# nk35jk/Chainer_Realtime_Multi-Person_Pose_Estimation

Measured on AMD Instinct MI355X. Metric: frames/sec end-to-end (CNN+PAF grouping) at 368×368, 1/2/4/8 MI355X, higher is better.
Workload: dtype bf16x3 (hi/lo split operands, f32 accumulate); 1 GPU; 368x368 frames, full PoseDetector.__call__ path (upload, resize+normalise, 92-conv CocoPoseNet in bf16x3: 3xBF16 split products, f32 accumulate, PAF post-process), batch of 232 frames per GPU per step; net_input=368x368, heatmap=320x320, maps=synthetic

## Files before the change

chainer_realtime_multi-person_pose_estimation_amd/_lib.py:

```python
import ctypes
import os

import numpy as np

_HERE = os.path.dirname(os.path.abspath(__file__))
LIB_PATH = os.path.join(_HERE, "libopenpose_hip%s.so" % (
    "." + os.environ["OP_LIB_VARIANT"] if os.environ.get("OP_LIB_VARIANT") else ""))

OP_OK, OP_ERR_INVALID, OP_ERR_HIP, OP_ERR_CAPACITY, OP_ERR_INDEX, OP_ERR_STATE, OP_ERR_TIMEOUT = range(7)
OP_COMM_ID_BYTES = 128
N_JOINTS, N_LIMBS, N_PAF, N_HEAT, N_LAYERS = 18, 19, 38, 19, 92

EXPORTED = (
    "op_last_error", "op_build_info", "op_default_params", "op_default_limits", "op_layer_info", "op_create", "op_destroy",
    "op_set_weights", "op_detect", "op_preprocess", "op_forward", "op_forward_stages", "op_forward_probe",
    "op_forward_probe_info", "op_resize_images", "op_compute_peaks",
    "op_compute_connections", "op_grouping", "op_postprocess", "op_stage_frames", "op_stage_maps",
    "op_use_staged_maps", "op_run_staged", "op_run_staged_graph", "op_graph_info", "op_synchronize", "op_fetch_result",
    "op_last_timing", "op_forward_flops", "op_profile_enable", "op_profile_read", "op_profile_reset",
    "op_set_precision", "op_get_precision", "op_fetch_results", "op_fetch_maps", "op_upload_frames", "op_upload_wait", "op_conv_census", "op_host_alloc", "op_host_free",
    "op_pack_results", "op_comm_unique_id", "op_comm_create", "op_comm_destroy", "op_comm_gather_results",
    "op_comm_wait", "op_comm_overflow", "op_comm_overflow_result", "op_detect_precise", "op_resize_cubic",
    "op_set_conv_algo", "op_set_stage_layout", "op_set_batch_invariant", "op_set_peak_mode", "op_profile_classes", "op_run_staged_precise",
    "op_cpm_layer_count", "op_cpm_layer_info", "op_cpm_create", "op_cpm_destroy", "op_cpm_set_weights",
# ... 309 lines not shown
        p.n_scales = len(sc)
        for i, v in enumerate(sc):
            p.inference_scales[i] = float(v)
    if "limbs_point" in d:
        for i, (a, b) in enumerate(d["limbs_point"]):
            p.limbs_point[i][0] = int(a)
            p.limbs_point[i][1] = int(b)
    return p


def layer_table():
    out = []
    name = ctypes.c_char_p()
    ci, co, k = ctypes.c_int32(), ctypes.c_int32(), ctypes.c_int32()
    for i in range(N_LAYERS):
        check(lib().op_layer_info(i, ctypes.byref(name), ctypes.byref(ci), ctypes.byref(co), ctypes.byref(k)))
        out.append((name.value.decode(), ci.value, co.value, k.value))
    return out


N_PROBE_POINTS = 46


def probe_table():
    out = []
    name = ctypes.c_char_p()
    ch, div = ctypes.c_int32(), ctypes.c_int32()
    for i in range(N_PROBE_POINTS):
        check(lib().op_forward_probe_info(i, ctypes.byref(name), ctypes.byref(ch), ctypes.byref(div)),
              "op_forward_probe_info")
        out.append((name.value.decode(), ch.value, div.value))
    return out


N_TRAIN_BUFFERS = 89


def train_buffer_table():
    out = []
    name = ctypes.c_char_p()
    ch, div = ctypes.c_int32(), ctypes.c_int32()
    for i in range(N_TRAIN_BUFFERS):
        check(lib().op_train_buffer_info(i, ctypes.byref(name), ctypes.byref(ch), ctypes.byref(div)),
              "op_train_buffer_info")
        out.append((name.value.decode(), ch.value, div.value))
    return out


CENSUS = {"7x7_splitk": 11, "7x7_other": 12, "3x3_w48": 13, "3x3_w32": 14, "3x3_pool": 15, "3x3_splitk": 16,
          "3x3_big": 17, "conv1_pair": 18, "3x3_r256": 19, "3x3_r128": 20, "3x3_r_pool": 21,
          "7x7_planar": 22, "7x7_frame_aligned": 23, "7x7_tight": 24,
          "cubic_fused": 25, "cubic_two_pass": 26,
          "cubic_rows": 28, "f32_lds": 29, "7x7_stag": 30, "7x7_plain_ring": 31,
          "7x7_q": 32, "7x7_circ": 33, "precise_side": 34, "7x7_q_iwg": 35, "7x7_lin": 36, "7x7_q_bpf": 37, "7x7_pers": 38}
CENSUS_SLOTS = 40


def conv_census(reset=False):
    a = (ctypes.c_int32 * CENSUS_SLOTS)()
    check(lib().op_conv_census(a, CENSUS_SLOTS, 1 if reset else 0), "op_conv_census")
    out = {"npx": {i: a[i] for i in range(1, 11) if a[i]}}
    out.update({k: a[v] for k, v in CENSUS.items()})
    return out


def forward_flops(h, w):
    return float(lib().op_forward_flops(int(h), int(w)))


class Context(object):

    def __init__(self, device=0, params=None, limits=None):
        L = lib()
        self._p = params if params is not None else default_params()
        self._l = limits if limits is not None else OpLimits()
        h = ctypes.c_void_p()
        check(L.op_create(ctypes.byref(self._p), ctypes.byref(self._l), int(device), ctypes.byref(h)), "op_create")
        self.h = h
        self.device = device

    def close(self):
        if getattr(self, "h", None) is not None and self.h.value:
            lib().op_destroy(self.h)
            self.h = None

    def __del__(self):
        try:
            self.close()
        except Exception:
            pass

    def set_precision(self, mode):
        check(lib().op_set_precision(self.h, PRECISION[mode]), "op_set_precision")

    def get_precision(self):
        m = ctypes.c_int32()
        check(lib().op_get_precision(self.h, ctypes.byref(m)), "op_get_precision")
        return {v: k for k, v in PRECISION.items()}[m.value]

    def set_weights(self, weights):
        table = layer_table()
        keep = []
        Wp = (ctypes.c_void_p * N_LAYERS)()
        bp = (ctypes.c_void_p * N_LAYERS)()
        for i, (name, ci, co, k) in enumerate(table):
            if name not in weights:
                raise KeyError("missing weights for layer %s" % name)
# ... 1077 lines not shown
```

chainer_realtime_multi-person_pose_estimation_amd/csrc/conv_big.hip:

```cpp
#include <atomic>
#include <array>
#include <map>
#include <mutex>
#include <tuple>
#include <cstdlib>
#include <vector>

#include "conv_big.hpp"
#include "conv_m16k.hpp"

namespace op {


template <int NPB, int KS, int PLANE_W>
__device__ __forceinline__ void big_taps(int nt, floatx16 (&acc)[2][NPB], const char* bp0, int hplane,
                                         const uint32_t (&qp)[(NPB + 1) / 2], const char* wb0, const char* wb1,
                                         int t, int pitch, int hi) {
  bf16x8g bh[2], bl[2], ah[2], al[2];
  auto q0 = [&](int pb) -> int { return (int)((qp[pb >> 1] >> (16 * (pb & 1))) & 0xffffu); };
  int toff = (t / KS) * pitch + (t - (t / KS) * KS);
  bh[0] = *(const bf16x8g*)(bp0 + (q0(0) + toff) * 16);
  bl[0] = *(const bf16x8g*)(bp0 + hplane + (q0(0) + toff) * 16);
#pragma unroll 1
  for (int u = 0; u < nt; ++u) {
// ... 889 lines not shown
      }
      if (plain_order) {
        tl.xpu = 0;
        tl.pair = 1;
      }
      tl.zeros = device_zeros();
      const char* trim_env = getenv("OP_M16_TRIM");
      tl.halo_trim = !(trim_env && atoi(trim_env) == 0);
      if (!tl.zeros) {
        set_error("conv_m16_bf16x3: conv_big_device_init was not called for this device");
        return OP_ERR_STATE;
      }
      *taken = 1;
      tl.ksplit = 1;
      tl.ws = nullptr;
      if (S > kMaxSplitK) S = 1;
      if (s.splitk && S > 1) {
        float* ws = splitk_ws(st, (size_t)S * s.groups * tl.total * cop_max);
        if (ws) {
          tl.ksplit = S;
          tl.ws = ws;
        }
      }
      const SplitConvGroup& g1 = s.groups > 1 ? g[1] : g[0];
      census_add(npx);
      if (tl.ksplit > 1) census_add(OP_CENSUS_7X7_SPLITK);
      if (s.in_planar) census_add(OP_CENSUS_7X7_PLANAR);
      if (tl.fa_tiles) census_add(OP_CENSUS_7X7_FRAME_ALIGNED);
      if (tl.pitch == s.w + 6) census_add(OP_CENSUS_7X7_TIGHT);
      const int rc = launch_m16_7x7(npx, st, s, g[0], g1, tl);
      if (rc != OP_OK) return rc;
      if (tl.ksplit > 1) {
        OP_AFTER_LAUNCH("conv_m16_bf16x3", st);
        const int64_t items = (int64_t)tl.total * (cop_max / 4);
        hipLaunchKernelGGL(conv_m16_splitk_reduce, dim3((unsigned)((items + 255) / 256), (unsigned)s.groups), dim3(256),
                           0, st, s, g[0], g1, tl);
      }
      OP_AFTER_LAUNCH("conv_m16_bf16x3", st);
      OP_HIP_CHECK(hipGetLastError());
      return OP_OK;
    }
    if (s.in_planar || s.out_planar) return OP_OK;
    if (raster_tiling(BigConfig{7, 6, 8, 128, 1, 1}, s.n, s.h, s.w, s.groups, cop_max, tl)) {
      if (plain_order) tl.xpu = 0;
      *taken = 1;
      return launch_big_t<7, 6, 8, 128, 1, false, true>(s, g, tl, st);
    }
    if (!big_tiling(BigConfig{7, 6, 8, 128, 1}, s.n, s.h, s.w, s.groups, cop_max, tl)) return OP_OK;
    if (plain_order) tl.xpu = 0;
    *taken = 1;
    return launch_big_t<7, 6, 8, 128, 1>(s, g, tl, st);
  }
  if (c128) {
    if (m16k_tiling(s, s.groups, cop_max, false, tl)) {
      const int rc = launch_conv_m16r(s, g, false, st, taken);
      if (rc != OP_OK || *taken) return rc;
      if (plain_order) tl.xpu = 0;
      *taken = 1;
      return launch_m16k(s, g, tl, false, st);
    }
    if (!big_tiling(BigConfig{3, 6, 4, 128, 0}, s.n, s.h, s.w, s.groups, cop_max, tl)) return OP_OK;
    if (plain_order) tl.xpu = 0;
    *taken = 1;
    return launch_big_t<3, 6, 4, 128, 0>(s, g, tl, st);
  }
  if (!big_tiling(BigConfig{3, 3, 4, 64, 0}, s.n, s.h, s.w, s.groups, cop_max, tl)) return OP_OK;
  if (plain_order) tl.xpu = 0;
  *taken = 1;
  return launch_big_t<3, 3, 4, 64, 0>(s, g, tl, st);
}

}

int op_conv_census(int32_t* counts, int32_t n, int32_t reset) {
  if (!counts || n < 1) return OP_ERR_INVALID;
  for (int i = 0; i < OP_CENSUS_SLOTS; ++i) {
    const int64_t v = reset ? op::g_census[i].exchange(0) : op::g_census[i].load();
    if (i < n) counts[i] = (int32_t)std::min<int64_t>(v, INT32_MAX);
  }
  for (int i = OP_CENSUS_SLOTS; i < n; ++i) counts[i] = 0;
  return OP_OK;
}
```

chainer_realtime_multi-person_pose_estimation_amd/csrc/conv_m16r.hip:

```cpp
#include <type_traits>

#include "conv_big.hpp"

namespace op {

__device__ __forceinline__ void dma16(const void* gsrc, uint32_t lds_byte) {
  asm volatile("s_mov_b32 m0, %1\n\ts_nop 0\n\tglobal_load_lds_dwordx4 %0, off" ::"v"(gsrc), "s"(lds_byte) : "memory");
}

template <int NW, int TCB, int TR, bool POOL, int CBW = 2>
__global__ __launch_bounds__(NW * 64, 2) void conv_m16r_bf16x3(SplitConvShape s, SplitConvGroup g0,
                                                                   SplitConvGroup g1, BigTiling tl) {
  static_assert(CBW == 2 || (CBW == 4 && NW == 4), "wave tiles: 32 channels, or 64 at NW 4");
  constexpr int PGN = CBW / 2;
  constexpr int NCS = NW / PGN;
  constexpr int NPT = TR * TCB;
  constexpr int NPX = NPT / PGN;
  constexpr int TC = 16 * TCB;
  constexpr int PITCH = TC + 2;
  constexpr int HROWS = TR + 2;
  constexpr int NH = (HROWS * PITCH + 63) / 64;
  constexpr int HPLANE = NH * 1024;
  constexpr int HBUF = 8 * HPLANE;
  constexpr int PIECES = 8 * NH / NW;
  constexpr int HSTEPS = 5;
  constexpr int PPS = (PIECES + HSTEPS - 1) / HSTEPS;
  constexpr int CW = NW * 32;
  static_assert((8 * NH) % NW == 0, "halo pieces split evenly over the waves");
  static_assert(NPT % PGN == 0 && (!POOL || (NPX % (2 * TCB)) == 0), "whole (pooled) row pairs per wave");
  static_assert(!POOL || (TR % 2 == 0), "pooled tiles hold whole row pairs");
  extern __shared__ __attribute__((aligned(16))) char lds[];

  const int lin = blockIdx.x;
  int unit, widx;
  if (tl.xpu) {
    const int xcd = lin & 7, slot = lin >> 3;
    const int P = tl.pair > 1 ? tl.pair : 1;
    const int su = xcd / tl.xpu, q = slot / P, xo = xcd - su * tl.xpu;
    unit = su * P + (slot - q * P);
    widx = tl.per_xcd > 0 ? xo * tl.per_xcd + q : q * tl.xpu + xo;
  } else {
    unit = lin / tl.per_unit;
    widx = lin - unit * tl.per_unit;
  }
  if (unit >= tl.units || widx >= tl.per_unit) return;
  const int grp = unit / tl.co_tiles;
  const int co0 = (unit - grp * tl.co_tiles) * CW;
  const SplitConvGroup g = grp == 0 ? g0 : g1;
  if (co0 >= g.cop) return;
  const int tpf = tl.tiles_y * tl.tiles_x;
  const int frame = widx / tpf;
  const int tix = widx - frame * tpf;
  const int ty = tix / tl.tiles_x;
  const int y0 = ty * TR, x0 = (tix - ty * tl.tiles_x) * TC;

  const int lane = threadIdx.x & 63;
  const int wave = __builtin_amdgcn_readfirstlane(threadIdx.x >> 6);
  const int cs = wave % NCS, pg = wave / NCS;
  const int l16 = lane & 15, kg = lane >> 4;
  const int csel = kg >> 1, khalf = kg & 1;
  const int wp_in = s.w + 2 * s.pin;
  const int hp_in = s.h + 2 * s.pin;
  const int64_t pix_bytes = (int64_t)s.cs_in * 4;
  const char* const fbase = (const char*)g.in + (int64_t)frame * hp_in * wp_in * pix_bytes;
  const uint32_t lds0 = (uint32_t)(size_t)(__attribute__((address_space(3))) char*)lds;

  const int64_t wplane = (int64_t)g.cop * 16;
  const int cw0 = co0 + cs * 16 * CBW;
  const char* const wlane = (const char*)g.w + ((int64_t)csel * 9 * 4 + 2 * khalf) * wplane + (int64_t)(cw0 + l16) * 16;
  const int ncp = s.c16 / 2;
  const int n_it = ncp * 9;
  typedef bf16x8g AFrag[2 * CBW];
  constexpr int NB = CBW == 2 ? 3 : 2;
  AFrag abuf[NB];
  auto load_a = [&](int it, AFrag& a) {
    if (it >= n_it) it = n_it - 1;
    const int cp = it / 9, t = it - cp * 9;
    const char* p = wlane + (int64_t)((2 * cp * 9 + t) * 4) * wplane;
#pragma unroll
    for (int cb = 0; cb < CBW; ++cb) {
      a[2 * cb] = *(const bf16x8g*)(p + cb * 256);
      a[2 * cb + 1] = *(const bf16x8g*)(p + wplane + cb * 256);
    }
  };

  auto halo_piece = [&](int cp, int buf, int k) {
    const int j = wave + k * NW;
    const int plane = j / NH, i = j - (j / NH) * NH;
    const int cj = plane >> 2, pl = plane & 3;
    const int slot = i * 64 + lane;
    const int hr = slot / PITCH, hc = slot - (slot / PITCH) * PITCH;
    const int yy = min(y0 - 1 + hr + s.pin, hp_in - 1), xx = min(x0 - 1 + hc + s.pin, wp_in - 1);
    const char* src = fbase + (int64_t)(yy * wp_in + xx) * pix_bytes + (2 * cp + cj) * 64 + pl * 16;
    dma16(src, lds0 + (uint32_t)(buf * HBUF + plane * HPLANE + i * 1024));
  };

  const int rows_here = min(TR, s.h - y0);
  const int cols_here = min(TC, s.w - x0);
  const int bl0 = (csel * 4 + 2 * khalf) * HPLANE + (l16 + pg * (NPX / TCB) * PITCH) * 16;

  floatx4 acc[CBW][NPX];
#pragma unroll
  for (int cb = 0; cb < CBW; ++cb)
#pragma unroll
    for (int pb = 0; pb < NPX; ++pb) acc[cb][pb] = floatx4{0.f, 0.f, 0.f, 0.f};

#pragma unroll
  for (int k = 0; k < PIECES; ++k) halo_piece(0, 0, k);
#pragma unroll
  for (int k = 0; k < NB - 1; ++k) load_a(k, abuf[k]);
  wait_vmcnt<0>();
  __builtin_amdgcn_s_barrier();
  asm volatile("" ::: "memory");

  auto chunk_pair = [&](int cp, auto parity) {
    constexpr int P = decltype(parity)::value;
    const int buf = cp & 1;
    const char* const hb = lds + buf * HBUF + bl0;
    const bool next = cp + 1 < ncp;
    constexpr int NBB = 2;
    auto boff = [&](int idx) {
      const int t1 = idx / NPX, pb1 = idx % NPX;
      return (((t1 / 3) + pb1 / TCB) * PITCH + (t1 % 3) + (pb1 % TCB) * 16) * 16;
    };
    bf16x8g bh[NBB], bl[NBB];
#pragma unroll
    for (int k = 0; k < NBB - 1; ++k) {
      bh[k] = *(const bf16x8g*)(hb + boff(k));
      bl[k] = *(const bf16x8g*)(hb + boff(k) + HPLANE);
    }
#pragma unroll
    for (int t = 0; t < 9; ++t) {
      const int it = cp * 9 + t;
      load_a(it + NB - 1, abuf[(9 * P + t + NB - 1) % NB]);
      if (t < HSTEPS && next) {
#pragma unroll
        for (int k = t * PPS; k < (t + 1) * PPS && k < PIECES; ++k) halo_piece(cp + 1, buf ^ 1, k);
      }
      const AFrag& a = abuf[(9 * P + t) % NB];
#pragma unroll
      for (int pb = 0; pb < NPX; ++pb) {
        const int idx = t * NPX + pb, cur = idx % NBB;
        if (idx + NBB - 1 < 9 * NPX) {
          const int o1 = boff(idx + NBB - 1);
          bh[(idx + NBB - 1) % NBB] = *(const bf16x8g*)(hb + o1);
          bl[(idx + NBB - 1) % NBB] = *(const bf16x8g*)(hb + o1 + HPLANE);
        }
        __builtin_amdgcn_sched_barrier(0);
#pragma unroll
        for (int cb = 0; cb < CBW; ++cb) {
          acc[cb][pb] = __builtin_amdgcn_mfma_f32_16x16x32_bf16(a[2 * cb], bh[cur], acc[cb][pb], 0, 0, 0);
          acc[cb][pb] = __builtin_amdgcn_mfma_f32_16x16x32_bf16(a[2 * cb], bl[cur], acc[cb][pb], 0, 0, 0);
          acc[cb][pb] = __builtin_amdgcn_mfma_f32_16x16x32_bf16(a[2 * cb + 1], bh[cur], acc[cb][pb], 0, 0, 0);
        }
      }
    }
    if (next) {
#ifdef M16R_WAIT8
      constexpr int kYounger = 8;
#else
      constexpr int kYounger = (9 - HSTEPS) * 2 * CBW;
#endif
      static_assert(kYounger >= 0 && kYounger <= 63, "vmcnt literal");
      wait_vmcnt<kYounger>();
      __builtin_amdgcn_s_barrier();
      asm volatile("" ::: "memory");
    }
  };
  if constexpr (NB == 3) {
    for (int cp = 0; cp < ncp; ++cp) chunk_pair(cp, std::integral_constant<int, 0>());
  } else {
    for (int cp = 0; cp < ncp; cp += 2) {
      chunk_pair(cp, std::integral_constant<int, 0>());
      if (cp + 1 < ncp) chunk_pair(cp + 1, std::integral_constant<int, 1>());
    }
  }
  wait_vmcnt<0>();

  if constexpr (POOL) {
    const int wp_out = s.w / 2 + 2 * s.pout;
    const int hp_out = s.h / 2 + 2 * s.pout;
#pragma unroll
    for (int pb = 0; pb < NPX; ++pb) {
      if ((pb / TCB) & 1) continue;
      const int r = pg * (NPX / TCB) + pb / TCB, c = (pb % TCB) * 16 + l16;
      const int y = y0 + r, x = x0 + c;
      const bool store = r < rows_here && c < cols_here && (l16 & 1) == 0;
      char* optr = (char*)g.out +
                   ((int64_t)(frame * hp_out + y / 2 + s.pout) * wp_out + (x / 2 + s.pout)) * (int64_t)s.cs_out * 4;
#pragma unroll
      for (int cb = 0; cb < CBW; ++cb) {
        const int co = cw0 + cb * 16 + 4 * kg;
        const bool live = co < g.cout_store;
        const floatx4 bv = live ? *(const floatx4*)(g.bias + co) : floatx4{0.f, 0.f, 0.f, 0.f};
        u16x4g vh, vl;
#pragma unroll
        for (int e = 0; e < 4; ++e) {
          float m = 0.0f;
#pragma unroll
          for (int k = 0; k < 2; ++k) {
            float f = acc[cb][pb + k * TCB][e] + bv[e];
            if (s.relu) f = f > 0.0f ? f : 0.0f;
            const __bf16 h16 = (__bf16)f;
            const float rc = (float)h16 + (float)(__bf16)(f - (float)h16);
            m = k == 0 ? rc : fmaxf(m, rc);
          }
          m = fmaxf(m, __shfl_xor(m, 1));
          const __bf16 h16 = (__bf16)m;
          const __bf16 l16v = (__bf16)(m - (float)h16);
          vh[e] = __builtin_bit_cast(unsigned short, h16);
          vl[e] = __builtin_bit_cast(unsigned short, l16v);
        }
        if (store && live) {
          char* d = optr + (co >> 3) * 32 + (co & 7) * 2;
          *(u16x4g*)d = vh;
          *(u16x4g*)(d + 16) = vl;
        }
      }
    }
    return;
  }

  const int wp_out = s.w + 2 * s.pout;
  const int hp_out = s.h + 2 * s.pout;
#pragma unroll
  for (int pb = 0; pb < NPX; ++pb) {
    const int r = pg * (NPX / TCB) + pb / TCB, c = (pb % TCB) * 16 + l16;
    const bool live = r < rows_here && c < cols_here;
    const int y = y0 + r, x = x0 + c;
    char* optr = (char*)g.out + ((int64_t)(frame * hp_out + y + s.pout) * wp_out + (x + s.pout)) * (int64_t)s.cs_out * 4;
    float* o32 = g.out32 ? g.out32 + ((int64_t)(frame * s.h + y) * s.w + x) * s.cs_out32 + g.out32_off : nullptr;
#pragma unroll
    for (int cb = 0; cb < CBW; ++cb) {
      const int co = cw0 + cb * 16 + 4 * kg;
      floatx4 v;
      uint32_t own[4], w[4];
      split_pair_swap(acc[cb][pb], co < g.cop ? *(const floatx4*)(g.bias + co) : floatx4{0.f, 0.f, 0.f, 0.f}, s.relu, v,
                      own, w);
      if (!live || co >= g.cout_store) continue;
      store_split_group(optr, co, kg, g.cout_store, own, w);
      if (o32) *(floatx4*)(o32 + co) = v;
    }
  }
}

template <int NW, int TCB, int TR, bool POOL, int CBW>
static int launch_t(const SplitConvShape& s, const SplitConvGroup& g0, const SplitConvGroup& g1, const BigTiling& tl,
                    hipStream_t st) {
  constexpr int PITCH = 16 * TCB + 2;
  constexpr int NH = ((TR + 2) * PITCH + 63) / 64;
  constexpr int LDS = 2 * 8 * NH * 1024;
  static_assert(LDS <= 160 * 1024 / (8 / NW), "workgroups per CU x LDS fits 160 KiB");
  static bool attr = false;
  if (!attr) {
    OP_HIP_CHECK(hipFuncSetAttribute((const void*)conv_m16r_bf16x3<NW, TCB, TR, POOL, CBW>,
                                     hipFuncAttributeMaxDynamicSharedMemorySize, LDS));
    attr = true;
  }
  const unsigned blocks = tl.xpu ? 8u * (unsigned)((tl.per_unit + tl.xpu - 1) / tl.xpu * std::max(tl.pair, 1))
                                 : (unsigned)(tl.units * tl.per_unit);
  hipLaunchKernelGGL((conv_m16r_bf16x3<NW, TCB, TR, POOL, CBW>), dim3(blocks), dim3(NW * 64), LDS, st, s, g0, g1, tl);
  return OP_OK;
}

int launch_conv_m16r(const SplitConvShape& s, const SplitConvGroup* g, bool pool, hipStream_t st, int* taken) {
  *taken = 0;
  static const int mode = getenv("OP_M16R") ? atoi(getenv("OP_M16R")) : 1;
  if (!mode || s.ks != 3 || s.pin < 1 || s.cs_in % 16 || (s.c16 & 1) || s.halo_mode != 4 || !s.regw) return OP_OK;
  int cop_max = 0;
  for (int i = 0; i < s.groups; ++i) {
    if (g[i].cop % 128 || g[i].cin_off % 16) return OP_OK;
    cop_max = std::max(cop_max, g[i].cop);
  }
  if (pool && (s.groups != 1 || (s.h & 1) || (s.w & 1) || !s.relu)) return OP_OK;
  const int nw = mode == 8 ? 8 : 4;
  if (nw == 8)
    for (int i = 0; i < s.groups; ++i)
      if (g[i].cop % 256) return OP_OK;
  constexpr int TCB = 3, TR = 4;
  BigTiling t{};
  t.tc = 16 * TCB;
  t.tr = TR;
  t.tiles_x = (s.w + t.tc - 1) / t.tc;
  t.tiles_y = (s.h + TR - 1) / TR;
  t.co_tiles = cop_max / (nw * 32);
  t.units = s.groups * t.co_tiles;
  t.per_unit = s.n * t.tiles_y * t.tiles_x;
  static const int pair_kb = getenv("OP_M16R_PAIR_KB") ? atoi(getenv("OP_M16R_PAIR_KB")) : 5000;
  const int64_t tile_wbytes = (int64_t)nw * 32 * s.c16 * 16 * 9 * 4;
  t.pair = 1;
  for (int p = t.co_tiles; p > 1; --p)
    if (t.co_tiles % p == 0 && p * tile_wbytes <= (int64_t)pair_kb * 1024 && (t.units / p) <= 8 &&
        8 % (t.units / p) == 0) {
      t.pair = p;
      break;
    }
  t.xpu = (t.units / t.pair <= 8 && 8 % (t.units / t.pair) == 0) ? 8 * t.pair / t.units : 0;
  if (!t.xpu) t.pair = 1;
  static const int xmaj = getenv("OP_M16R_XMAJ") ? atoi(getenv("OP_M16R_XMAJ")) : 1;
  t.per_xcd = xmaj && t.xpu ? (t.per_unit + t.xpu - 1) / t.xpu : 0;
  const int64_t wgs = (int64_t)t.units * t.per_unit;
  if (wgs < (nw == 8 ? 2 * 256 : 4 * 256)) return OP_OK;
  *taken = 1;
  const SplitConvGroup& g1 = s.groups > 1 ? g[1] : g[0];
  census_add(pool ? OP_CENSUS_3X3_R_POOL : nw == 8 ? OP_CENSUS_3X3_R256 : OP_CENSUS_3X3_R128);
  static const int cbw = getenv("OP_M16R_CBW") ? atoi(getenv("OP_M16R_CBW")) : 2;
  int rc;
  if (nw == 8)
    rc = pool ? launch_t<8, TCB, TR, true, 2>(s, g[0], g1, t, st) : launch_t<8, TCB, TR, false, 2>(s, g[0], g1, t, st);
  else if (cbw == 4)
    rc = pool ? launch_t<4, TCB, TR, true, 4>(s, g[0], g1, t, st) : launch_t<4, TCB, TR, false, 4>(s, g[0], g1, t, st);
  else
    rc = pool ? launch_t<4, TCB, TR, true, 2>(s, g[0], g1, t, st) : launch_t<4, TCB, TR, false, 2>(s, g[0], g1, t, st);
  if (rc != OP_OK) return rc;
  OP_AFTER_LAUNCH("conv_m16r_bf16x3", st);
  OP_HIP_CHECK(hipGetLastError());
  return OP_OK;
}

}
```

include/openpose_hip.h:

```cpp
#ifndef OPENPOSE_HIP_H
#define OPENPOSE_HIP_H

#include <stdint.h>

#ifdef __cplusplus
extern "C" {
#endif

#define OP_OK 0
#define OP_ERR_INVALID 1
#define OP_ERR_HIP 2
#define OP_ERR_CAPACITY 3
#define OP_ERR_INDEX 4
#define OP_ERR_STATE 5
#define OP_ERR_TIMEOUT 6

#define OP_N_JOINTS 18
#define OP_N_LIMBS 19
#define OP_N_PAF 38
#define OP_N_HEAT 19
#define OP_N_LAYERS 92
#define OP_MAX_SCALES 8

typedef struct op_params {
// ... 99 lines not shown
int op_stage_frames(op_ctx* ctx, const uint8_t* frames, int32_t n, int32_t h, int32_t w);
int op_upload_frames(op_ctx* ctx, const uint8_t* frames, int32_t n, int32_t h, int32_t w);
int op_upload_wait(op_ctx* ctx);
int op_host_alloc(size_t bytes, void** p);
int op_host_free(void* p);
int op_stage_maps(op_ctx* ctx, const float* maps, int32_t n, int32_t mh, int32_t mw);
int op_use_staged_maps(op_ctx* ctx, int32_t enable);
int op_run_staged(op_ctx* ctx);
int op_run_staged_precise(op_ctx* ctx);
int op_run_staged_graph(op_ctx* ctx);
int op_graph_info(op_ctx* ctx, int32_t* nodes, int32_t* kernels, int32_t* memsets, int32_t* memcpys,
                  int32_t* host_nodes);
int op_synchronize(op_ctx* ctx);
int op_fetch_result(op_ctx* ctx, int32_t frame, double* poses, double* scores, int32_t cap, op_frame_result* res);

int op_fetch_results(op_ctx* ctx, int32_t first, int32_t n, double* poses, double* scores, int32_t cap,
                     op_frame_result* res);

int op_fetch_maps(op_ctx* ctx, int32_t first, int32_t n, float* pafs, float* heatmaps, int32_t* mh, int32_t* mw);
int op_last_timing(op_ctx* ctx, double* conv_ms, double* post_ms, double* total_ms);
int op_profile_enable(op_ctx* ctx, int32_t enable);
int op_profile_read(op_ctx* ctx, int32_t cls, double* ms, int64_t* launches, double* flops, double* bytes);
int op_profile_reset(op_ctx* ctx);
#define OP_PROFILE_CLASSES 7
int op_profile_classes(op_ctx* ctx, int32_t mask);

#define OP_CENSUS_7X7_SPLITK 11
#define OP_CENSUS_7X7_OTHER 12
#define OP_CENSUS_3X3_W48 13
#define OP_CENSUS_3X3_W32 14
#define OP_CENSUS_3X3_POOL 15
#define OP_CENSUS_3X3_SPLITK 16
#define OP_CENSUS_3X3_BIG 17
#define OP_CENSUS_CONV1_PAIR 18
#define OP_CENSUS_3X3_R256 19
#define OP_CENSUS_3X3_R128 20
#define OP_CENSUS_3X3_R_POOL 21
#define OP_CENSUS_7X7_PLANAR 22
#define OP_CENSUS_7X7_FRAME_ALIGNED 23
#define OP_CENSUS_7X7_TIGHT 24
#define OP_CENSUS_CUBIC_FUSED 25
#define OP_CENSUS_CUBIC_TWO_PASS 26
#define OP_CENSUS_CUBIC_ROWS 28
#define OP_CENSUS_F32_LDS 29
#define OP_CENSUS_7X7_STAG 30
#define OP_CENSUS_7X7_PLAIN_RING 31
#define OP_CENSUS_7X7_Q 32
#define OP_CENSUS_7X7_CIRC 33
#define OP_CENSUS_PRECISE_SIDE 34
#define OP_CENSUS_7X7_Q_IWG 35
#define OP_CENSUS_7X7_LIN 36
#define OP_CENSUS_7X7_Q_BPF 37
#define OP_CENSUS_7X7_PERS 38
#define OP_CENSUS_SLOTS 40
int op_conv_census(int32_t* counts, int32_t n, int32_t reset);

double op_forward_flops(int32_t h, int32_t w);

int op_pack_results(op_ctx* ctx, int32_t first, int32_t n, int32_t max_persons, int64_t frame_base,
                    int32_t frame_stride, void* host_records);
#define OP_COMM_ID_BYTES 128
typedef struct op_comm op_comm;
int op_comm_unique_id(uint8_t* id);
int op_comm_create(op_ctx* ctx, int32_t world, int32_t rank, const uint8_t* id, double timeout_s, op_comm** out);
int op_comm_destroy(op_comm* comm);
int op_comm_gather_results(op_comm* comm, op_ctx* ctx, int32_t first, int32_t n, int32_t max_persons,
                           int64_t frame_base, int32_t frame_stride);
int op_comm_wait(op_comm* comm, double timeout_s, const void** records, int32_t* n_frames, int64_t* rec_bytes);
int op_comm_overflow(op_comm* comm, op_ctx* ctx, int32_t* frames, int32_t* reasons, int32_t cap, int32_t* count);
int op_comm_overflow_result(op_comm* comm, op_ctx* ctx, int32_t frame, double* poses, double* scores, int32_t cap,
                            op_frame_result* res);

#define OP_ARCH_FACENET 1
#define OP_ARCH_HANDNET 2
typedef struct op_cpm_ctx op_cpm_ctx;
int op_cpm_layer_count(int32_t arch);
int op_cpm_layer_info(int32_t arch, int32_t index, const char** name, int32_t* ci, int32_t* co, int32_t* ksize);
int op_cpm_create(int32_t arch, int32_t device, op_cpm_ctx** out);
int op_cpm_destroy(op_cpm_ctx* ctx);
int op_cpm_set_weights(op_cpm_ctx* ctx, const float* const* W, const float* const* b);
int op_cpm_forward(op_cpm_ctx* ctx, const float* x, int32_t n, int32_t h, int32_t w, float* maps);
#define OP_CPM_PROBE_HI 256
int op_cpm_probe_info(int32_t arch, int32_t point, const char** name, int32_t* channels, int32_t* divisor);
int op_cpm_forward_probe(op_cpm_ctx* ctx, const float* x, int32_t n, int32_t h, int32_t w, int32_t point,
                         int32_t frame0, int32_t nframes, float* out, int64_t out_floats);
int op_cpm_peaks(op_cpm_ctx* ctx, const float* heatmaps, int32_t c, int32_t h, int32_t w, float thresh,
                 int32_t flip, double* keypoints, int32_t* found);
int op_cpm_detect(op_cpm_ctx* ctx, const uint8_t* bgr, int32_t h, int32_t w, int64_t row_stride, float thresh,
                  int32_t flip_maps, double* keypoints, int32_t* found);
int op_cpm_detect_batch(op_cpm_ctx* ctx, int32_t n, const uint8_t* const* bgr, const int32_t* h, const int32_t* w,
                        const int64_t* row_stride, float thresh, const int32_t* flip_maps, double* keypoints,
                        int32_t* found);
int op_cpm_set_batch_invariant(op_cpm_ctx* ctx, int32_t enable);
int op_cpm_detect_rois(op_cpm_ctx* ctx, int32_t n_frames, const uint8_t* const* bgr, const int32_t* fh,
                       const int32_t* fw, const int64_t* row_stride, int32_t n, const int32_t* roi_frame,
                       const int32_t* roi_box, const int32_t* roi_mirror, float thresh, double* keypoints,
                       int32_t* found);
int op_cpm_set_roi_group_bytes(op_cpm_ctx* ctx, int64_t bytes);
int op_cpm_roi_stats(op_cpm_ctx* ctx, int64_t out[4]);
int op_cpm_detect_rois_staged(op_cpm_ctx* cpm, op_ctx* ctx, int32_t first, int32_t n_frames, int32_t n,
                              const int32_t* roi_frame, const int32_t* roi_box, const int32_t* roi_mirror,
                              float thresh, double* keypoints, int32_t* found);
int op_cpm_set_roi_batch(op_cpm_ctx* cpm, int32_t rois);

typedef struct op_train_ctx op_train_ctx;
int op_train_create(int32_t device, int32_t n, int32_t h, int32_t w, op_train_ctx** out);
// ... 175 lines not shown
```

Baseline: 1971 frames/s.

## Add persistent tile-walking mode to m16r 3x3 conv with cross-tile halo prefetch

Restructures the m16r bf16x3 3x3 conv kernel so a workgroup can loop over several tiles of the same output-channel unit. The last chunk pair of one tile prefetches the next tile's halo and wraps the weight prefetch, which overlaps tile start-up with the previous tile's compute. Bias loads are hoisted out of the epilogue, and halo offsets are precomputed per tile so the DMA uses a scalar base plus a 32-bit vector offset. Walking only turns on when OP_M16R_WALK=1, so the default path keeps one tile per block but still runs the reworked loop, epilogue and addressing. The change also removes the CBW=4 env option and adds a guard against planes of 4 GiB or more.

```diff
diff --git a/chainer_realtime_multi-person_pose_estimation_amd/_lib.py b/chainer_realtime_multi-person_pose_estimation_amd/_lib.py
--- a/chainer_realtime_multi-person_pose_estimation_amd/_lib.py
+++ b/chainer_realtime_multi-person_pose_estimation_amd/_lib.py
@@ -385,7 +385,8 @@
           "7x7_planar": 22, "7x7_frame_aligned": 23, "7x7_tight": 24,
           "cubic_fused": 25, "cubic_two_pass": 26,
           "cubic_rows": 28, "f32_lds": 29, "7x7_stag": 30, "7x7_plain_ring": 31,
-          "7x7_q": 32, "7x7_circ": 33, "precise_side": 34, "7x7_q_iwg": 35, "7x7_lin": 36, "7x7_q_bpf": 37, "7x7_pers": 38}
+          "7x7_q": 32, "7x7_circ": 33, "precise_side": 34, "7x7_q_iwg": 35, "7x7_lin": 36, "7x7_q_bpf": 37, "7x7_pers": 38,
+          "3x3_r_walk": 39}
 CENSUS_SLOTS = 40
 
 
diff --git a/chainer_realtime_multi-person_pose_estimation_amd/csrc/conv_big.hip b/chainer_realtime_multi-person_pose_estimation_amd/csrc/conv_big.hip
--- a/chainer_realtime_multi-person_pose_estimation_amd/csrc/conv_big.hip
+++ b/chainer_realtime_multi-person_pose_estimation_amd/csrc/conv_big.hip
@@ -965,9 +965,12 @@
     return launch_big_t<7, 6, 8, 128, 1>(s, g, tl, st);
   }
   if (c128) {
-    if (m16k_tiling(s, s.groups, cop_max, false, tl)) {
+    const bool m16k = m16k_tiling(s, s.groups, cop_max, false, tl);
+    if (m16k || getenv("OP_M16R_MIN_WG")) {
       const int rc = launch_conv_m16r(s, g, false, st, taken);
       if (rc != OP_OK || *taken) return rc;
+    }
+    if (m16k) {
       if (plain_order) tl.xpu = 0;
       *taken = 1;
       return launch_m16k(s, g, tl, false, st);
diff --git a/chainer_realtime_multi-person_pose_estimation_amd/csrc/conv_m16r.hip b/chainer_realtime_multi-person_pose_estimation_amd/csrc/conv_m16r.hip
--- a/chainer_realtime_multi-person_pose_estimation_amd/csrc/conv_m16r.hip
+++ b/chainer_realtime_multi-person_pose_estimation_amd/csrc/conv_m16r.hip
@@ -4,9 +4,20 @@
 
 namespace op {
 
-__device__ __forceinline__ void dma16(const void* gsrc, uint32_t lds_byte) {
-  asm volatile("s_mov_b32 m0, %1\n\ts_nop 0\n\tglobal_load_lds_dwordx4 %0, off" ::"v"(gsrc), "s"(lds_byte) : "memory");
+__device__ __forceinline__ void dma16(const void* sbase, uint32_t voff, uint32_t lds_byte) {
+  asm volatile("s_mov_b32 m0, %2\n\ts_nop 0\n\tglobal_load_lds_dwordx4 %0, %1" ::"v"(voff), "s"(sbase), "s"(lds_byte)
+               : "memory");
 }
+
+#if M16R_STAMPS
+__device__ unsigned long long g_m16r_st[6];
+#define M16R_T() __builtin_amdgcn_s_memtime()
+#endif
+
+struct M16rTile {
+  int frame, y0, x0;
+  const char* fbase;
+};
 
 template <int NW, int TCB, int TR, bool POOL, int CBW = 2>
 __global__ __launch_bounds__(NW * 64, 2) void conv_m16r_bf16x3(SplitConvShape s, SplitConvGroup g0,
@@ -31,38 +42,53 @@
   static_assert(!POOL || (TR % 2 == 0), "pooled tiles hold whole row pairs");
   extern __shared__ __attribute__((aligned(16))) char lds[];
 
-  const int lin = blockIdx.x;
-  int unit, widx;
-  if (tl.xpu) {
-    const int xcd = lin & 7, slot = lin >> 3;
-    const int P = tl.pair > 1 ? tl.pair : 1;
-    const int su = xcd / tl.xpu, q = slot / P, xo = xcd - su * tl.xpu;
-    unit = su * P + (slot - q * P);
-    widx = tl.per_xcd > 0 ? xo * tl.per_xcd + q : q * tl.xpu + xo;
-  } else {
-    unit = lin / tl.per_unit;
-    widx = lin - unit * tl.per_unit;
-  }
-  if (unit >= tl.units || widx >= tl.per_unit) return;
+#if M16R_STAMPS
+  const unsigned long long st_t0 = M16R_T();
+  unsigned long long st_epi = 0, st_tiles = 0;
+#endif
+  const int wp_in = s.w + 2 * s.pin;
+  const int hp_in = s.h + 2 * s.pin;
+  const int64_t pix_bytes = (int64_t)s.cs_in * 4;
+  auto slot_tile = [&](int lin, int& unit) {
+    int widx;
+    if (tl.xpu) {
+      const int xcd = lin & 7, slot = lin >> 3;
+      const int P = tl.pair > 1 ? tl.pair : 1;
+      const int su = xcd / tl.xpu, q = slot / P, xo = xcd - su * tl.xpu;
+      unit = su * P + (slot - q * P);
+      widx = tl.per_xcd > 0 ? xo * tl.per_xcd + q : q * tl.xpu + xo;
+    } else {
+      unit = lin / tl.per_unit;
+      widx = lin - unit * tl.per_unit;
+    }
+    return lin < tl.pers_blocks && unit < tl.units && widx < tl.per_unit ? widx : -1;
+  };
+  int lin = blockIdx.x, unit, unit_n;
+  int widx = slot_tile(lin, unit);
+  if (widx < 0) return;
   const int grp = unit / tl.co_tiles;
   const int co0 = (unit - grp * tl.co_tiles) * CW;
   const SplitConvGroup g = grp == 0 ? g0 : g1;
   if (co0 >= g.cop) return;
   const int tpf = tl.tiles_y * tl.tiles_x;
-  const int frame = widx / tpf;
-  const int tix = widx - frame * tpf;
-  const int ty = tix / tl.tiles_x;
-  const int y0 = ty * TR, x0 = (tix - ty * tl.tiles_x) * TC;
+  auto tile_at = [&](int widx) {
+    M16rTile t;
+    t.frame = widx / tpf;
+    const int tix = widx - t.frame * tpf;
+    const int ty = tix / tl.tiles_x;
+    t.y0 = ty * TR;
+    t.x0 = (tix - ty * tl.tiles_x) * TC;
+    t.fbase = (const char*)g.in + (int64_t)t.frame * hp_in * wp_in * pix_bytes;
+    return t;
+  };
+  M16rTile cur = tile_at(widx), nxt = cur;
+  bool more = false;
 
   const int lane = threadIdx.x & 63;
   const int wave = __builtin_amdgcn_readfirstlane(threadIdx.x >> 6);
   const int cs = wave % NCS, pg = wave / NCS;
   const int l16 = lane & 15, kg = lane >> 4;
   const int csel = kg >> 1, khalf = kg & 1;
-  const int wp_in = s.w + 2 * s.pin;
-  const int hp_in = s.h + 2 * s.pin;
-  const int64_t pix_bytes = (int64_t)s.cs_in * 4;
-  const char* const fbase = (const char*)g.in + (int64_t)frame * hp_in * wp_in * pix_bytes;
   const uint32_t lds0 = (uint32_t)(size_t)(__attribute__((address_space(3))) char*)lds;
 
   const int64_t wplane = (int64_t)g.cop * 16;
@@ -74,7 +100,7 @@
   constexpr int NB = CBW == 2 ? 3 : 2;
   AFrag abuf[NB];
   auto load_a = [&](int it, AFrag& a) {
-    if (it >= n_it) it = n_it - 1;
+    if (it >= n_it) it -= n_it;
     const int cp = it / 9, t = it - cp * 9;
     const char* p = wlane + (int64_t)((2 * cp * 9 + t) * 4) * wplane;
 #pragma unroll
@@ -83,20 +109,32 @@
       a[2 * cb + 1] = *(const bf16x8g*)(p + wplane + cb * 256);
     }
   };
-
+  auto landed = [&](AFrag& a) {
+#pragma unroll
+    for (int i = 0; i < 2 * CBW; ++i) asm volatile("" : "+v"(a[i]));
+  };
+
+  const char* hbase;
+  uint32_t hoff[PIECES];
+  auto halo_tile = [&](const M16rTile& tt) {
+    hbase = tt.fbase;
+#pragma unroll
+    for (int k = 0; k < PIECES; ++k) {
+      const int j = wave + k * NW;
+      const int i = j - (j / NH) * NH;
+      const int slot = i * 64 + lane;
+      const int hr = slot / PITCH, hc = slot - (slot / PITCH) * PITCH;
+      const int yy = min(tt.y0 - 1 + hr + s.pin, hp_in - 1), xx = min(tt.x0 - 1 + hc + s.pin, wp_in - 1);
+      hoff[k] = (uint32_t)(yy * wp_in + xx) * (uint32_t)pix_bytes;
+    }
+  };
   auto halo_piece = [&](int cp, int buf, int k) {
     const int j = wave + k * NW;
     const int plane = j / NH, i = j - (j / NH) * NH;
     const int cj = plane >> 2, pl = plane & 3;
-    const int slot = i * 64 + lane;
-    const int hr = slot / PITCH, hc = slot - (slot / PITCH) * PITCH;
-    const int yy = min(y0 - 1 + hr + s.pin, hp_in - 1), xx = min(x0 - 1 + hc + s.pin, wp_in - 1);
-    const char* src = fbase + (int64_t)(yy * wp_in + xx) * pix_bytes + (2 * cp + cj) * 64 + pl * 16;
-    dma16(src, lds0 + (uint32_t)(buf * HBUF + plane * HPLANE + i * 1024));
-  };
-
-  const int rows_here = min(TR, s.h - y0);
-  const int cols_here = min(TC, s.w - x0);
+    dma16(hbase + ((2 * cp + cj) * 64 + pl * 16), hoff[k], lds0 + (uint32_t)(buf * HBUF + plane * HPLANE + i * 1024));
+  };
+
   const int bl0 = (csel * 4 + 2 * khalf) * HPLANE + (l16 + pg * (NPX / TCB) * PITCH) * 16;
 
   floatx4 acc[CBW][NPX];
@@ -105,19 +143,34 @@
 #pragma unroll
     for (int pb = 0; pb < NPX; ++pb) acc[cb][pb] = floatx4{0.f, 0.f, 0.f, 0.f};
 
+  halo_tile(cur);
 #pragma unroll
   for (int k = 0; k < PIECES; ++k) halo_piece(0, 0, k);
 #pragma unroll
   for (int k = 0; k < NB - 1; ++k) load_a(k, abuf[k]);
+  floatx4 bias[CBW];
+#pragma unroll
+  for (int cb = 0; cb < CBW; ++cb) {
+    const int co = cw0 + cb * 16 + 4 * kg;
+    bias[cb] = co < (POOL ? g.cout_store : g.cop) ? *(const floatx4*)(g.bias + co) : floatx4{0.f, 0.f, 0.f, 0.f};
+  }
   wait_vmcnt<0>();
+#pragma unroll
+  for (int k = 0; k < NB - 1; ++k) landed(abuf[k]);
+#pragma unroll
+  for (int cb = 0; cb < CBW; ++cb) asm volatile("" : "+v"(bias[cb]));
   __builtin_amdgcn_s_barrier();
   asm volatile("" ::: "memory");
-
-  auto chunk_pair = [&](int cp, auto parity) {
-    constexpr int P = decltype(parity)::value;
-    const int buf = cp & 1;
+#if M16R_STAMPS
+  const unsigned long long st_t1 = M16R_T();
+#endif
+
+  auto chunk_pair = [&](int buf, bool next, int cp, auto first, auto last_pair, auto parity)
+                        __attribute__((always_inline)) {
+    constexpr int PAR = decltype(parity)::value;
+    constexpr bool last = decltype(last_pair)::value;
     const char* const hb = lds + buf * HBUF + bl0;
-    const bool next = cp + 1 < ncp;
+    const int hcp = last ? 0 : cp + 1;
     constexpr int NBB = 2;
     auto boff = [&](int idx) {
       const int t1 = idx / NPX, pb1 = idx % NPX;
@@ -132,15 +185,15 @@
 #pragma unroll
     for (int t = 0; t < 9; ++t) {
       const int it = cp * 9 + t;
-      load_a(it + NB - 1, abuf[(9 * P + t + NB - 1) % NB]);
+      load_a(it + NB - 1, abuf[(9 * PAR + t + NB - 1) % NB]);
       if (t < HSTEPS && next) {
 #pragma unroll
-        for (int k = t * PPS; k < (t + 1) * PPS && k < PIECES; ++k) halo_piece(cp + 1, buf ^ 1, k);
+        for (int k = t * PPS; k < (t + 1) * PPS && k < PIECES; ++k) halo_piece(hcp, buf ^ 1, k);
       }
-      const AFrag& a = abuf[(9 * P + t) % NB];
+      const AFrag& a = abuf[(9 * PAR + t) % NB];
 #pragma unroll
       for (int pb = 0; pb < NPX; ++pb) {
-        const int idx = t * NPX + pb, cur = idx % NBB;
+        const int idx = t * NPX + pb, cur_b = idx % NBB;
         if (idx + NBB - 1 < 9 * NPX) {
           const int o1 = boff(idx + NBB - 1);
           bh[(idx + NBB - 1) % NBB] = *(const bf16x8g*)(hb + o1);
@@ -149,13 +202,17 @@
         __builtin_amdgcn_sched_barrier(0);
 #pragma unroll
         for (int cb = 0; cb < CBW; ++cb) {
-          acc[cb][pb] = __builtin_amdgcn_mfma_f32_16x16x32_bf16(a[2 * cb], bh[cur], acc[cb][pb], 0, 0, 0);
-          acc[cb][pb] = __builtin_amdgcn_mfma_f32_16x16x32_bf16(a[2 * cb], bl[cur], acc[cb][pb], 0, 0, 0);
-          acc[cb][pb] = __builtin_amdgcn_mfma_f32_16x16x32_bf16(a[2 * cb + 1], bh[cur], acc[cb][pb], 0, 0, 0);
+          acc[cb][pb] = __builtin_amdgcn_mfma_f32_16x16x32_bf16(a[2 * cb], bh[cur_b], acc[cb][pb], 0, 0, 0);
+          acc[cb][pb] = __builtin_amdgcn_mfma_f32_16x16x32_bf16(a[2 * cb], bl[cur_b], acc[cb][pb], 0, 0, 0);
+          acc[cb][pb] = __builtin_amdgcn_mfma_f32_16x16x32_bf16(a[2 * cb + 1], bh[cur_b], acc[cb][pb], 0, 0, 0);
         }
       }
     }
-    if (next) {
+    if constexpr (last) {
+      wait_vmcnt<0>();
+#pragma unroll
+      for (int k = 0; k < NB - 1; ++k) landed(abuf[(9 * PAR + 9 + k) % NB]);
+    } else {
 #ifdef M16R_WAIT8
       constexpr int kYounger = 8;
 #else
@@ -163,90 +220,145 @@
 #endif
       static_assert(kYounger >= 0 && kYounger <= 63, "vmcnt literal");
       wait_vmcnt<kYounger>();
+    }
+    if (next) {
       __builtin_amdgcn_s_barrier();
       asm volatile("" ::: "memory");
     }
   };
-  if constexpr (NB == 3) {
-    for (int cp = 0; cp < ncp; ++cp) chunk_pair(cp, std::integral_constant<int, 0>());
-  } else {
-    for (int cp = 0; cp < ncp; cp += 2) {
-      chunk_pair(cp, std::integral_constant<int, 0>());
-      if (cp + 1 < ncp) chunk_pair(cp + 1, std::integral_constant<int, 1>());
-    }
-  }
-  wait_vmcnt<0>();
-
-  if constexpr (POOL) {
-    const int wp_out = s.w / 2 + 2 * s.pout;
-    const int hp_out = s.h / 2 + 2 * s.pout;
-#pragma unroll
-    for (int pb = 0; pb < NPX; ++pb) {
-      if ((pb / TCB) & 1) continue;
-      const int r = pg * (NPX / TCB) + pb / TCB, c = (pb % TCB) * 16 + l16;
-      const int y = y0 + r, x = x0 + c;
-      const bool store = r < rows_here && c < cols_here && (l16 & 1) == 0;
-      char* optr = (char*)g.out +
-                   ((int64_t)(frame * hp_out + y / 2 + s.pout) * wp_out + (x / 2 + s.pout)) * (int64_t)s.cs_out * 4;
-#pragma unroll
-      for (int cb = 0; cb < CBW; ++cb) {
-        const int co = cw0 + cb * 16 + 4 * kg;
-        const bool live = co < g.cout_store;
-        const floatx4 bv = live ? *(const floatx4*)(g.bias + co) : floatx4{0.f, 0.f, 0.f, 0.f};
-        u16x4g vh, vl;
-#pragma unroll
-        for (int e = 0; e < 4; ++e) {
-          float m = 0.0f;
-#pragma unroll
-          for (int k = 0; k < 2; ++k) {
-            float f = acc[cb][pb + k * TCB][e] + bv[e];
-            if (s.relu) f = f > 0.0f ? f : 0.0f;
-            const __bf16 h16 = (__bf16)f;
-            const float rc = (float)h16 + (float)(__bf16)(f - (float)h16);
-            m = k == 0 ? rc : fmaxf(m, rc);
+
+  auto epilogue = [&](const M16rTile& tt) __attribute__((always_inline)) {
+    const int rows_here = min(TR, s.h - tt.y0);
+    const int cols_here = min(TC, s.w - tt.x0);
+    if constexpr (POOL) {
+      const int wp_out = s.w / 2 + 2 * s.pout;
+      const int hp_out = s.h / 2 + 2 * s.pout;
+#pragma unroll
+      for (int pb = 0; pb < NPX; ++pb) {
+        if ((pb / TCB) & 1) continue;
+        const int r = pg * (NPX / TCB) + pb / TCB, c = (pb % TCB) * 16 + l16;
+        const int y = tt.y0 + r, x = tt.x0 + c;
+        const bool store = r < rows_here && c < cols_here && (l16 & 1) == 0;
+        char* optr = (char*)g.out + ((int64_t)(tt.frame * hp_out + y / 2 + s.pout) * wp_out + (x / 2 + s.pout)) *
+                                        (int64_t)s.cs_out * 4;
+#pragma unroll
+        for (int cb = 0; cb < CBW; ++cb) {
+          const int co = cw0 + cb * 16 + 4 * kg;
+          const bool live = co < g.cout_store;
+          const floatx4 bv = bias[cb];
+          u16x4g vh, vl;
+#pragma unroll
+          for (int e = 0; e < 4; ++e) {
+            float m = 0.0f;
+#pragma unroll
+            for (int k = 0; k < 2; ++k) {
+              float f = acc[cb][pb + k * TCB][e] + bv[e];
+              if (s.relu) f = f > 0.0f ? f : 0.0f;
+              const __bf16 h16 = (__bf16)f;
+              const float rc = (float)h16 + (float)(__bf16)(f - (float)h16);
+              m = k == 0 ? rc : fmaxf(m, rc);
+            }
+            m = fmaxf(m, __shfl_xor(m, 1));
+            const __bf16 h16 = (__bf16)m;
+            const __bf16 l16v = (__bf16)(m - (float)h16);
+            vh[e] = __builtin_bit_cast(unsigned short, h16);
+            vl[e] = __builtin_bit_cast(unsigned short, l16v);
           }
-          m = fmaxf(m, __shfl_xor(m, 1));
-          const __bf16 h16 = (__bf16)m;
-          const __bf16 l16v = (__bf16)(m - (float)h16);
-          vh[e] = __builtin_bit_cast(unsigned short, h16);
-          vl[e] = __builtin_bit_cast(unsigned short, l16v);
-        }
-        if (store && live) {
-          char* d = optr + (co >> 3) * 32 + (co & 7) * 2;
-          *(u16x4g*)d = vh;
-          *(u16x4g*)(d + 16) = vl;
+          if (store && live) {
+            char* d = optr + (co >> 3) * 32 + (co & 7) * 2;
+            *(u16x4g*)d = vh;
+            *(u16x4g*)(d + 16) = vl;
+          }
         }
       }
-    }
-    return;
-  }
-
-  const int wp_out = s.w + 2 * s.pout;
-  const int hp_out = s.h + 2 * s.pout;
-#pragma unroll
-  for (int pb = 0; pb < NPX; ++pb) {
-    const int r = pg * (NPX / TCB) + pb / TCB, c = (pb % TCB) * 16 + l16;
-    const bool live = r < rows_here && c < cols_here;
-    const int y = y0 + r, x = x0 + c;
-    char* optr = (char*)g.out + ((int64_t)(frame * hp_out + y + s.pout) * wp_out + (x + s.pout)) * (int64_t)s.cs_out * 4;
-    float* o32 = g.out32 ? g.out32 + ((int64_t)(frame * s.h + y) * s.w + x) * s.cs_out32 + g.out32_off : nullptr;
-#pragma unroll
-    for (int cb = 0; cb < CBW; ++cb) {
-      const int co = cw0 + cb * 16 + 4 * kg;
-      floatx4 v;
-      uint32_t own[4], w[4];
-      split_pair_swap(acc[cb][pb], co < g.cop ? *(const floatx4*)(g.bias + co) : floatx4{0.f, 0.f, 0.f, 0.f}, s.relu, v,
-                      own, w);
-      if (!live || co >= g.cout_store) continue;
-      store_split_group(optr, co, kg, g.cout_store, own, w);
-      if (o32) *(floatx4*)(o32 + co) = v;
-    }
-  }
+    } else {
+      const int wp_out = s.w + 2 * s.pout;
+      const int hp_out = s.h + 2 * s.pout;
+#pragma unroll
+      for (int pb = 0; pb < NPX; ++pb) {
+        const int r = pg * (NPX / TCB) + pb / TCB, c = (pb % TCB) * 16 + l16;
+        const bool live = r < rows_here && c < cols_here;
+        const int y = tt.y0 + r, x = tt.x0 + c;
+        char* optr =
+            (char*)g.out + ((int64_t)(tt.frame * hp_out + y + s.pout) * wp_out + (x + s.pout)) * (int64_t)s.cs_out * 4;
+        float* o32 =
+            g.out32 ? g.out32 + ((int64_t)(tt.frame * s.h + y) * s.w + x) * s.cs_out32 + g.out32_off : nullptr;
+#pragma unroll
+        for (int cb = 0; cb < CBW; ++cb) {
+          const int co = cw0 + cb * 16 + 4 * kg;
+          floatx4 v;
+          uint32_t own[4], w[4];
+          split_pair_swap(acc[cb][pb], bias[cb], s.relu, v, own, w);
+          if (!live || co >= g.cout_store) continue;
+          store_split_group(optr, co, kg, g.cout_store, own, w);
+          if (o32) *(floatx4*)(o32 + co) = v;
+        }
+      }
+    }
+  };
+
+  int gp = 0;
+  auto pair = [&](int cp, auto first, auto last_pair) __attribute__((always_inline)) {
+    constexpr bool last = decltype(last_pair)::value;
+    if constexpr (last) {
+      lin += gridDim.x;
+      const int widx_n = slot_tile(lin, unit_n);
+      more = widx_n >= 0 && unit_n == unit;
+      if (more) {
+        nxt = tile_at(widx_n);
+        halo_tile(nxt);
+      }
+    }
+    const bool next = !last || more;
+    if constexpr (NB == 3) {
+      chunk_pair(gp & 1, next, cp, first, last_pair, std::integral_constant<int, 0>());
+    } else {
+      if (gp & 1) chunk_pair(1, next, cp, first, last_pair, std::integral_constant<int, 1>());
+      else chunk_pair(0, next, cp, first, last_pair, std::integral_constant<int, 0>());
+    }
+    ++gp;
+  };
+  for (;;) {
+    int cp0 = 0, cpl = ncp - 1;
+    asm volatile("" : "+s"(cp0), "+s"(cpl));
+    pair(cp0, std::true_type(), std::false_type());
+    for (int cp = 1; cp + 1 < ncp; ++cp) pair(cp, std::false_type(), std::false_type());
+    pair(cpl, std::false_type(), std::true_type());
+#if M16R_STAMPS
+    const unsigned long long st_e0 = M16R_T();
+#endif
+    epilogue(cur);
+#if M16R_STAMPS
+    st_epi += M16R_T() - st_e0;
+    ++st_tiles;
+#endif
+    if (!more) break;
+#pragma unroll
+    for (int cb = 0; cb < CBW; ++cb)
+#pragma unroll
+      for (int pb = 0; pb < NPX; ++pb) acc[cb][pb] = floatx4{0.f, 0.f, 0.f, 0.f};
+    cur = nxt;
+  }
+#if M16R_STAMPS
+  const unsigned long long st_t2 = M16R_T();
+#endif
+  wait_vmcnt<0>();
+#if M16R_STAMPS
+  const unsigned long long st_t3 = M16R_T();
+  if (lane == 0) {
+    atomicAdd(&g_m16r_st[0], st_t3 - st_t0);
+    atomicAdd(&g_m16r_st[1], st_t1 - st_t0);
+    atomicAdd(&g_m16r_st[2], st_epi);
+    atomicAdd(&g_m16r_st[3], 1ull);
+    atomicAdd(&g_m16r_st[4], st_tiles);
+    atomicAdd(&g_m16r_st[5], st_t3 - st_t2);
+  }
+#endif
 }
 
 template <int NW, int TCB, int TR, bool POOL, int CBW>
-static int launch_t(const SplitConvShape& s, const SplitConvGroup& g0, const SplitConvGroup& g1, const BigTiling& tl,
-                    hipStream_t st) {
+static int launch_t(const SplitConvShape& s, const SplitConvGroup& g0, const SplitConvGroup& g1, BigTiling tl,
+                    int walk_wgs, hipStream_t st, int* walked) {
   constexpr int PITCH = 16 * TCB + 2;
   constexpr int NH = ((TR + 2) * PITCH + 63) / 64;
   constexpr int LDS = 2 * 8 * NH * 1024;
@@ -259,20 +371,29 @@
   }
   const unsigned blocks = tl.xpu ? 8u * (unsigned)((tl.per_unit + tl.xpu - 1) / tl.xpu * std::max(tl.pair, 1))
                                  : (unsigned)(tl.units * tl.per_unit);
-  hipLaunchKernelGGL((conv_m16r_bf16x3<NW, TCB, TR, POOL, CBW>), dim3(blocks), dim3(NW * 64), LDS, st, s, g0, g1, tl);
+  tl.pers_blocks = (int)blocks;
+  unsigned grid = blocks;
+  if (walk_wgs > 0 && tl.xpu) {
+    const unsigned row = 8u * (unsigned)std::max(tl.pair, 1);
+    grid = std::min(blocks, std::max((unsigned)walk_wgs / row, 1u) * row);
+  }
+  *walked = grid < blocks;
+  hipLaunchKernelGGL((conv_m16r_bf16x3<NW, TCB, TR, POOL, CBW>), dim3(grid), dim3(NW * 64), LDS, st, s, g0, g1, tl);
   return OP_OK;
 }
 
 int launch_conv_m16r(const SplitConvShape& s, const SplitConvGroup* g, bool pool, hipStream_t st, int* taken) {
   *taken = 0;
   static const int mode = getenv("OP_M16R") ? atoi(getenv("OP_M16R")) : 1;
-  if (!mode || s.ks != 3 || s.pin < 1 || s.cs_in % 16 || (s.c16 & 1) || s.halo_mode != 4 || !s.regw) return OP_OK;
+  if (!mode || s.ks != 3 || s.pin < 1 || s.cs_in % 16 || (s.c16 & 1) || s.c16 < 4 || s.halo_mode != 4 || !s.regw)
+    return OP_OK;
   int cop_max = 0;
   for (int i = 0; i < s.groups; ++i) {
     if (g[i].cop % 128 || g[i].cin_off % 16) return OP_OK;
     cop_max = std::max(cop_max, g[i].cop);
   }
   if (pool && (s.groups != 1 || (s.h & 1) || (s.w & 1) || !s.relu)) return OP_OK;
+  if ((int64_t)(s.h + 2 * s.pin) * (s.w + 2 * s.pin) * s.cs_in * 4 >= (1ll << 32)) return OP_OK;
   const int nw = mode == 8 ? 8 : 4;
   if (nw == 8)
     for (int i = 0; i < s.groups; ++i)
@@ -300,21 +421,50 @@
   static const int xmaj = getenv("OP_M16R_XMAJ") ? atoi(getenv("OP_M16R_XMAJ")) : 1;
   t.per_xcd = xmaj && t.xpu ? (t.per_unit + t.xpu - 1) / t.xpu : 0;
   const int64_t wgs = (int64_t)t.units * t.per_unit;
-  if (wgs < (nw == 8 ? 2 * 256 : 4 * 256)) return OP_OK;
+  const char* e = getenv("OP_M16R_MIN_WG");
+  if (wgs < (e && atoi(e) > 0 ? atoi(e) : nw == 8 ? 2 * 256 : 4 * 256)) return OP_OK;
+  static int n_cu = 0;
+  if (!n_cu) {
+    int dev = 0;
+    OP_HIP_CHECK(hipGetDevice(&dev));
+    OP_HIP_CHECK(hipDeviceGetAttribute(&n_cu, hipDeviceAttributeMultiprocessorCount, dev));
+  }
+  int walk_wgs = (e = getenv("OP_M16R_WALK")) && atoi(e) == 1 ? n_cu * (8 / nw) : 0;
+  if (walk_wgs && (e = getenv("OP_M16R_WALK_WGS")) && atoi(e) > 0) walk_wgs = std::min(walk_wgs, atoi(e));
+  int walked = 0;
   *taken = 1;
   const SplitConvGroup& g1 = s.groups > 1 ? g[1] : g[0];
   census_add(pool ? OP_CENSUS_3X3_R_POOL : nw == 8 ? OP_CENSUS_3X3_R256 : OP_CENSUS_3X3_R128);
-  static const int cbw = getenv("OP_M16R_CBW") ? atoi(getenv("OP_M16R_CBW")) : 2;
   int rc;
+#define M16R_LAUNCH(NW_, POOL_, CBW_) launch_t<NW_, TCB, TR, POOL_, CBW_>(s, g[0], g1, t, walk_wgs, st, &walked)
   if (nw == 8)
-    rc = pool ? launch_t<8, TCB, TR, true, 2>(s, g[0], g1, t, st) : launch_t<8, TCB, TR, false, 2>(s, g[0], g1, t, st);
-  else if (cbw == 4)
-    rc = pool ? launch_t<4, TCB, TR, true, 4>(s, g[0], g1, t, st) : launch_t<4, TCB, TR, false, 4>(s, g[0], g1, t, st);
+    rc = pool ? M16R_LAUNCH(8, true, 2) : M16R_LAUNCH(8, false, 2);
   else
-    rc = pool ? launch_t<4, TCB, TR, true, 2>(s, g[0], g1, t, st) : launch_t<4, TCB, TR, false, 2>(s, g[0], g1, t, st);
+    rc = pool ? M16R_LAUNCH(4, true, 2) : M16R_LAUNCH(4, false, 2);
+#undef M16R_LAUNCH
   if (rc != OP_OK) return rc;
+  if (walked) census_add(OP_CENSUS_3X3_R_WALK);
   OP_AFTER_LAUNCH("conv_m16r_bf16x3", st);
   OP_HIP_CHECK(hipGetLastError());
+#if M16R_STAMPS
+  static const bool dump = getenv("OP_M16R_STAMPS") != nullptr;
+  hipStreamCaptureStatus cst = hipStreamCaptureStatusNone;
+  if (dump && hipStreamIsCapturing(st, &cst) == hipSuccess && cst == hipStreamCaptureStatusNone) {
+    unsigned long long h[6];
+    OP_HIP_CHECK(hipStreamSynchronize(st));
+    OP_HIP_CHECK(hipMemcpyFromSymbol(h, HIP_SYMBOL(g_m16r_st), sizeof(h)));
+    const unsigned long long z[6] = {};
+    OP_HIP_CHECK(hipMemcpyToSymbol(HIP_SYMBOL(g_m16r_st), z, sizeof(z)));
+    const double w = (double)h[0], tiles = (double)h[4], steps = 9.0 * (s.c16 / 2);
+    const double per_step = (w - h[1] - h[2] - h[5]) / (tiles * steps);
+    fprintf(stderr,
+            "M16R_STAMPS n %d %dx%d c16 %d cop %d pool %d walked %d | waves %llu tiles/wave %.2f | per tile cycles %.0f | "
+            "before first pair %.4f pair loop %.4f epilogue %.4f final drain %.4f | K-step %.0f cycles, fixed phase "
+            "%.2f K-steps per tile\n",
+            s.n, s.h, s.w, s.c16, cop_max, (int)pool, walked, h[3], tiles / h[3], w / tiles, h[1] / w,
+            (w - h[1] - h[2] - h[5]) / w, h[2] / w, h[5] / w, per_step, (h[1] + h[2] + h[5]) / tiles / per_step);
+  }
+#endif
   return OP_OK;
 }
 
diff --git a/include/openpose_hip.h b/include/openpose_hip.h
--- a/include/openpose_hip.h
+++ b/include/openpose_hip.h
@@ -175,6 +175,7 @@
 #define OP_CENSUS_7X7_LIN 36
 #define OP_CENSUS_7X7_Q_BPF 37
 #define OP_CENSUS_7X7_PERS 38
+#define OP_CENSUS_3X3_R_WALK 39
 #define OP_CENSUS_SLOTS 40
 int op_conv_census(int32_t* counts, int32_t n, int32_t reset);
 
```

Result: no change. 1975 frames/s, median of 3 (+0.2%).
